# kokkos/kokkos-kernels

Hardware: NVIDIA B200
Metric: spmv_fp64_gflops (higher is better)
Workload: dtype f64

## Files before the change

include/b200sparse.h:

```cpp
#ifndef B200SPARSE_H_
#define B200SPARSE_H_

#include <stdint.h>

#ifdef __cplusplus
extern "C" {
#endif

typedef enum {
  B200SP_OK = 0,
  B200SP_ERR_INVALID_ARGUMENT = 1,
  B200SP_ERR_CUDA = 2,
  B200SP_ERR_STATE = 3,
  B200SP_ERR_OVERFLOW = 4,
  B200SP_ERR_ALLOC = 5
} b200sp_status;

typedef enum {
  B200SP_SPMV_DEFAULT = 0,
  B200SP_SPMV_FAST_SETUP = 1,
  B200SP_SPMV_MERGE_PATH = 2
} b200sp_spmv_algo;

typedef struct b200sp_spmv_plan b200sp_spmv_plan;
// ... 248 lines not shown
int b200sp_gmres_bsr_f64_i32(b200sp_bsr_plan* plan_A, void* stream, int mb, int64_t nnzb, int bs, const int* row_ptr,
                             const int* col_idx, const double* vals, b200sp_bsr_plan* plan_M, int64_t nnzb_M,
                             const int* row_ptr_M, const int* col_idx_M, const double* vals_M, const double* b, double* x,
                             int m, double tol, int max_restart, int ortho, int* num_iters, double* end_rel_res,
                             int* conv_flag);
int b200sp_gmres_bsr_f32_i32(b200sp_bsr_plan* plan_A, void* stream, int mb, int64_t nnzb, int bs, const int* row_ptr,
                             const int* col_idx, const float* vals, b200sp_bsr_plan* plan_M, int64_t nnzb_M,
                             const int* row_ptr_M, const int* col_idx_M, const float* vals_M, const float* b, float* x, int m,
                             float tol, int max_restart, int ortho, int* num_iters, float* end_rel_res, int* conv_flag);

int64_t b200sp_launch_count(void);
const char* b200sp_spmv_last_kernel(const b200sp_spmv_plan* plan);
int b200sp_spmv_plan_invalidate(b200sp_spmv_plan* plan, void* stream);

int b200sp_spmv_plan_tune(b200sp_spmv_plan* plan, int cfg, int lanes_per_row, int ctas_per_sm);
#ifdef __cplusplus
}
#endif
#endif
```

kokkos-kernels_b200/_lib.py:

```python
import ctypes as C
import os

HERE = os.path.dirname(os.path.abspath(__file__))
LIBDIR = os.path.join(HERE, "lib")
SPARSE_SO = os.path.join(LIBDIR, "libb200sparse.so")
MATGEN_SO = os.path.join(LIBDIR, "libb200matgen.so")

i32, i64, f32, f64, vp, cp = C.c_int, C.c_int64, C.c_float, C.c_double, C.c_void_p, C.c_char
u64 = C.c_uint64

SPARSE_API = {
    "b200sp_last_error_string": (C.c_char_p, []),
    "b200sp_version": (i32, []),
    "b200sp_device_ok": (i32, []),
    "b200sp_spmv_plan_create": (i32, [C.POINTER(vp), i32]),
    "b200sp_spmv_plan_destroy": (i32, [vp, vp]),
    "b200sp_spmv_plan_set_option": (i32, [vp, i32, i32]),
    "b200sp_spmv_f64_i32": (i32, [vp, vp, cp, i32, i32, i64, f64, vp, vp, vp, vp, f64, vp]),
    "b200sp_spmv_f32_i32": (i32, [vp, vp, cp, i32, i32, i64, f32, vp, vp, vp, vp, f32, vp]),
    "b200sp_gs2_plan_create": (i32, [C.POINTER(vp)]),
    "b200sp_gs2_plan_destroy": (i32, [vp, vp]),
    "b200sp_gs2_plan_set": (i32, [vp, i32, f64]),
    "b200sp_gs2_symbolic_i32": (i32, [vp, vp, i32, i32, vp, vp]),
    "b200sp_gs2_numeric_f64_i32": (i32, [vp, vp, i32, i32, vp, vp, vp, vp]),
# ... 8 lines not shown
    "b200sp_sptrsv_solve_f64_i32": (i32, [vp, vp, i32, vp, vp, vp, vp, vp]),
    "b200sp_sptrsv_solve_f32_i32": (i32, [vp, vp, i32, vp, vp, vp, vp, vp]),
    "b200sp_spmv_hostvec_flush": (i32, [vp, vp]),
    "b200sp_spmv64_plan_create": (i32, [C.POINTER(vp), i32]),
    "b200sp_spmv64_plan_destroy": (i32, [vp, vp]),
    "b200sp_spmv64_plan_set_window": (i32, [vp, i64]),
    "b200sp_spmv64_plan_windows": (i32, [vp]),
    "b200sp_spmv64_last_kernel": (C.c_char_p, [vp]),
    "b200sp_spmv_f64_i64": (i32, [vp, vp, cp, i64, i64, i64, f64, vp, vp, i32, vp, vp, f64, vp]),
    "b200sp_spmv_f32_i64": (i32, [vp, vp, cp, i64, i64, i64, f32, vp, vp, i32, vp, vp, f32, vp]),
    "b200sp_spmm_f64_i64": (i32, [vp, vp, cp, i64, i64, i64, i32, f64, vp, vp, i32, vp, vp, i64, i32, f64, vp, i64, i32]),
    "b200sp_spmm_f32_i64": (i32, [vp, vp, cp, i64, i64, i64, i32, f32, vp, vp, i32, vp, vp, i64, i32, f32, vp, i64, i32]),
    "b200sp_spmv_scatter_f64_i32": (i32, [vp, vp, i32, i32, i64, f64, vp, vp, vp, vp, vp, i32, C.POINTER(vp)]),
    "b200sp_spmv_forward_f64_i32": (i32, [vp, vp, i32, i32, i64, f64, vp, vp, vp, vp, vp, vp]),
    "b200sp_spmv_plan_invalidate": (i32, [vp, vp]),
    "b200sp_peer_push": (i32, [vp, vp, i64, i32, C.POINTER(vp)]),
    "b200sp_peer_push_async": (i32, [vp, C.POINTER(vp), i32, C.POINTER(vp), vp, i64]),
    "b200sp_peer_join": (i32, [vp, C.POINTER(vp), i32]),
    "b200sp_multicast_push": (i32, [vp, vp, vp, i64, i32]),
    "b200sp_peer_push_sm": (i32, [vp, vp, i64, i32, C.POINTER(vp), i32]),
    "b200sp_spmv_hostvec_f64_i32": (i32, [vp, vp, cp, i32, i32, i64, f64, vp, vp, vp, vp, f64, vp]),
    "b200sp_spmm_f64_i32": (i32, [vp, vp, cp, i32, i32, i64, i32, f64, vp, vp, vp, vp, i64, i32, f64, vp, i64, i32]),
    "b200sp_spmm_f32_i32": (i32, [vp, vp, cp, i32, i32, i64, i32, f32, vp, vp, vp, vp, i64, i32, f32, vp, i64, i32]),
    "b200sp_spgemm_plan_create": (i32, [C.POINTER(vp)]),
    "b200sp_spgemm_plan_destroy": (i32, [vp, vp]),
    "b200sp_spgemm_symbolic_i32": (i32, [vp, vp, i32, i32, i32, vp, vp, vp, vp, vp, C.POINTER(i64), C.POINTER(i32)]),
    "b200sp_spgemm_numeric_f64_i32": (i32, [vp, vp, i32, i32, i32, vp, vp, vp, vp, vp, vp, vp, vp, vp]),
    "b200sp_spgemm_numeric_f32_i32": (i32, [vp, vp, i32, i32, i32, vp, vp, vp, vp, vp, vp, vp, vp, vp]),
    "b200sp_spgemm_jacobi_f64_i32": (i32, [vp, vp, i32, i32, i32, vp, vp, vp, vp, vp, vp, vp, vp, vp, f64, vp]),
    "b200sp_spgemm_jacobi_f32_i32": (i32, [vp, vp, i32, i32, i32, vp, vp, vp, vp, vp, vp, vp, vp, vp, f32, vp]),
# ... 112 lines not shown
```

kokkos-kernels_b200/csrc/spmv.cu:

```cuda
#include "common.cuh"
#include "tile_ring.cuh"
#include "spmm_items.h"
#include <stdarg.h>
#include <stdlib.h>
#include <string.h>
#include <algorithm>
#include <mutex>

namespace b200sp {

static thread_local char g_err[512] = "";
std::atomic<long long> g_launches{0};

void set_error(const char* fmt, ...) {
  va_list ap;
  va_start(ap, fmt);
  vsnprintf(g_err, sizeof(g_err), fmt, ap);
  va_end(ap);
}

int sm_count() {
  static int cached[64];
  static std::once_flag once;
  std::call_once(once, [] { memset(cached, 0, sizeof(cached)); });
// ... 449 lines not shown
          }
#pragma unroll
          for (int u = 0; u < UNR; ++u) xv[u] = (j0 + u * LPR < jend) ? ldg(x + c[u]) : S(0);
#pragma unroll
          for (int u = 0; u < UNR; ++u) sum += av[u] * xv[u];
        }
        sum = subwarp_sum<LPR>(sum);
        if (valid && !is_long && sl == 0) store_y(y, r, sum, alpha, beta, ex);
      }
      __syncwarp();
      if (lane == 0) mbar_arrive(&sm.empty[stage]);
    }
  }
}

struct TileCfg {
  int cap, stages, nw;
};
static const TileCfg kCfgs[] = {
    {2048, 4, 8},
    {4096, 4, 16},
    {4096, 3, 8},
    {1024, 6, 8},
    {2048, 3, 16},
    {2048, 3, 24},
    {2048, 3, 31},
    {1024, 5, 16},
    {2048, 4, 16},
    {2048, 3, 16},
    {4096, 3, 31},
// ... 92 lines not shown
  int algo = B200SP_SPMV_DEFAULT;
  int cfg = -1, lpr = -1, ctas_per_sm = -1;
  const int* key_row_ptr = nullptr;
  int key_m = -1, key_n = -1;
  int64_t key_nnz = -1;
  int key_cfg = -1;
  int4* tiles = nullptr;
  int n_tiles = 0;
  int T = 0, LMAX = 0;
  int* long_rows = nullptr;
  int* n_long = nullptr;
  int* n_long_host = nullptr;
  cudaEvent_t n_long_event = nullptr;
  bool n_long_known = false;
  int long_cap = 0;
  void* dx = nullptr;
  void* dy = nullptr;
  size_t dx_bytes = 0, dy_bytes = 0;
  void* xt = nullptr;
  void* yt = nullptr;
  size_t xt_bytes = 0, yt_bytes = 0;
  int* chunk_row = nullptr;
  int n_chunks = 0, chunk_q = 0;
  const int* chunk_key = nullptr;
  int chunk_m = -1;
  int64_t chunk_nnz = -1;
  int4* r1_segs = nullptr;
  int* r1_n_seg = nullptr;
  int2* r1_row_seg = nullptr;
  void* r1_partial = nullptr;
// ... 53 lines not shown
  if (p->r1_segs) cudaFreeAsync(p->r1_segs, st);
  if (p->r1_n_seg) cudaFreeAsync(p->r1_n_seg, st);
  if (p->r1_row_seg) cudaFreeAsync(p->r1_row_seg, st);
  if (p->r1_partial) cudaFreeAsync(p->r1_partial, st);
  p->r1_segs = nullptr;
  p->r1_n_seg = nullptr;
  p->r1_row_seg = nullptr;
  p->r1_partial = nullptr;
  p->r1_built = false;
  p->tiles = nullptr;
  p->long_rows = nullptr;
  p->n_long = nullptr;
  p->n_tiles = 0;
  p->n_long_known = false;
  p->key_row_ptr = nullptr;
}

static void plan_release_mm(b200sp_spmv_plan* p, cudaStream_t st) {
  void* ptrs[] = {p->mm_tiles, p->mm_long_rows, p->mm_n_long, p->mm_segs, p->mm_n_seg};
  for (void* q : ptrs)
    if (q) cudaFreeAsync(q, st);
  p->mm_tiles = nullptr;
  p->mm_long_rows = nullptr;
  p->mm_n_long = nullptr;
  p->mm_segs = nullptr;
  p->mm_n_seg = nullptr;
  p->mm_key_row_ptr = nullptr;
  void* iptrs[] = {p->mmi.items, p->mmi.multi, p->mmi.partial};
  for (void* q : iptrs)
    if (q) cudaFreeAsync(q, st);
  p->mmi = b200sp::MMItems();
}

b200sp::MMItems* plan_mm_items(b200sp_spmv_plan* p) { return &p->mmi; }

template <typename S>
static int plan_analyse(b200sp_spmv_plan* p, cudaStream_t st, int cfg, int m, int n, int64_t nnz,
                        const int* row_ptr) {
  if (p->key_row_ptr == row_ptr && p->key_m == m && p->key_n == n && p->key_nnz == nnz &&
      p->key_cfg == cfg && p->tiles)
    return B200SP_OK;
  plan_release_analysis(p, st);
  const TileCfg c = kCfgs[cfg];
  p->LMAX = c.cap / 4;
  p->T = c.cap - p->LMAX - 8;
  p->n_tiles = (int)(nnz / p->T) + 1;
  p->long_cap = (int)(nnz / (p->LMAX + 1)) + 1;
  B200SP_CUDA_TRY(cudaMallocAsync((void**)&p->tiles, sizeof(int4) * (size_t)p->n_tiles, st));
  B200SP_CUDA_TRY(cudaMallocAsync((void**)&p->long_rows, sizeof(int) * (size_t)p->long_cap, st));
  B200SP_CUDA_TRY(cudaMallocAsync((void**)&p->n_long, sizeof(int), st));
  B200SP_CUDA_TRY(cudaMemsetAsync(p->n_long, 0, sizeof(int), st));
  build_tiles_kernel<<<(p->n_tiles + 255) / 256, 256, 0, st>>>(m, row_ptr, p->n_tiles, p->T, c.cap, p->tiles);
  B200SP_LAUNCH_CHECK();
  find_long_rows_kernel<<<std::max(1, std::min((m + 255) / 256, sm_count() * 8)), 256, 0, st>>>(m, row_ptr, p->LMAX,
                                                                                                p->long_rows, p->n_long);
  B200SP_LAUNCH_CHECK();
  if (!p->n_long_host) B200SP_CUDA_TRY(cudaMallocHost((void**)&p->n_long_host, sizeof(int)));
  if (!p->n_long_event) B200SP_CUDA_TRY(cudaEventCreateWithFlags(&p->n_long_event, cudaEventDisableTiming));
  *p->n_long_host = -1;
  B200SP_CUDA_TRY(cudaMemcpyAsync(p->n_long_host, p->n_long, sizeof(int), cudaMemcpyDeviceToHost, st));
  B200SP_CUDA_TRY(cudaEventRecord(p->n_long_event, st));
  p->n_long_known = false;
  p->key_row_ptr = row_ptr;
  p->key_m = m;
  p->key_n = n;
  p->key_nnz = nnz;
  p->key_cfg = cfg;
  p->at_calls = 0;
  p->at_choice = -1;
  return B200SP_OK;
}

int plan_mv_scratch(b200sp_spmv_plan* p, cudaStream_t st, size_t xt_bytes, size_t yt_bytes, void** xt, void** yt) {
  if (xt_bytes > p->xt_bytes) {
    if (p->xt) cudaFreeAsync(p->xt, st);
    p->xt = nullptr;
    p->xt_bytes = 0;
    B200SP_CUDA_TRY(cudaMallocAsync(&p->xt, xt_bytes, st));
// ... 126 lines not shown
      kf<<<grid, (NW + 1) * 32, smem, st>>>(m, nnz, hi - lo, p->LMAX, p->tiles + lo, row_ptr, col_idx, vals, x, y, alpha, beta,
                                            p->extra);
      launched = true;
    }
  }
  if (!launched)
    kern<<<grid, (NW + 1) * 32, smem, st>>>(m, nnz, hi - lo, p->LMAX, p->tiles + lo, row_ptr, col_idx, vals, x, y,
                                            alpha, beta, direct_extra(p->extra));
  B200SP_LAUNCH_CHECK();
  snprintf(p->last_kernel, sizeof(p->last_kernel), "tile<%s,LPR=%d,NW=%d,STAGES=%d,CAP=%d,UNR=%d>grid=%d",
           sizeof(S) == 8 ? "f64" : "f32", LPR, NW, STAGES, CAP, UNR, grid);
  return B200SP_OK;
}

template <typename S, int LPR>
static int launch_tile_cfg(b200sp_spmv_plan* p, int cfg, cudaStream_t st, int m, int64_t nnz,
                           const int* row_ptr, const int* col_idx, const S* vals, const S* x, S* y,
                           S alpha, S beta) {
  switch (cfg) {
    case 0: return launch_tile<S, LPR, 8, 4, 2048>(p, st, m, nnz, row_ptr, col_idx, vals, x, y, alpha, beta);
    case 1: return launch_tile<S, LPR, 16, 4, 4096>(p, st, m, nnz, row_ptr, col_idx, vals, x, y, alpha, beta);
    case 2: return launch_tile<S, LPR, 8, 3, 4096>(p, st, m, nnz, row_ptr, col_idx, vals, x, y, alpha, beta);
    case 3: return launch_tile<S, LPR, 8, 6, 1024>(p, st, m, nnz, row_ptr, col_idx, vals, x, y, alpha, beta);
    case 4: return launch_tile<S, LPR, 16, 3, 2048>(p, st, m, nnz, row_ptr, col_idx, vals, x, y, alpha, beta);
    case 5: return launch_tile<S, LPR, 24, 3, 2048>(p, st, m, nnz, row_ptr, col_idx, vals, x, y, alpha, beta);
    case 6: return launch_tile<S, LPR, 31, 3, 2048>(p, st, m, nnz, row_ptr, col_idx, vals, x, y, alpha, beta);
    case 7: return launch_tile<S, LPR, 16, 5, 1024>(p, st, m, nnz, row_ptr, col_idx, vals, x, y, alpha, beta);
    case 8: return launch_tile<S, LPR, 16, 4, 2048>(p, st, m, nnz, row_ptr, col_idx, vals, x, y, alpha, beta);
    case 9: return launch_tile<S, LPR, 16, 3, 2048, 4>(p, st, m, nnz, row_ptr, col_idx, vals, x, y, alpha, beta);
    case 10: return launch_tile<S, LPR, 31, 3, 4096>(p, st, m, nnz, row_ptr, col_idx, vals, x, y, alpha, beta);
// ... 126 lines not shown
      case 8: spmv_transpose_kernel<S, 8><<<blocks, 256, 0, st>>>(m, row_ptr, col_idx, vals, x, y, alpha); break;
      case 16: spmv_transpose_kernel<S, 16><<<blocks, 256, 0, st>>>(m, row_ptr, col_idx, vals, x, y, alpha); break;
      default: spmv_transpose_kernel<S, 32><<<blocks, 256, 0, st>>>(m, row_ptr, col_idx, vals, x, y, alpha); break;
    }
    B200SP_LAUNCH_CHECK();
    if (p) snprintf(p->last_kernel, sizeof(p->last_kernel), "transpose<%s,LPR=%d>", sizeof(S) == 8 ? "f64" : "f32", lpr);
    return B200SP_OK;
  }

  const bool aligned = (((uintptr_t)vals | (uintptr_t)col_idx | (uintptr_t)row_ptr) & 15u) == 0;
  const bool use_tile = p && p->algo != B200SP_SPMV_FAST_SETUP && aligned &&
                        (nnz >= 32768 || p->cfg >= 0);
  if (!use_tile) return launch_vector<S>(p, st, (p && p->lpr > 0) ? p->lpr : lpr_auto, m, row_ptr, col_idx, vals, x, y, alpha, beta);

  const int cfg = p->cfg >= 0 ? p->cfg : 8;
  int rc = plan_analyse<S>(p, st, cfg, m, n, nnz, row_ptr);
  if (rc) return rc;
  const int lpr = p->lpr > 0 ? p->lpr : lpr_auto;
  const bool autotune = p->cfg < 0 && p->range_hi < 0 && p->extra.n == 0 && getenv("B200SP_NO_AUTOTUNE") == nullptr;
  int phase = -1;
  bool use_vec = false;
  if (autotune) {
    if (p->at_choice < 0 && p->at_calls >= 3 && cudaEventQuery(p->at_ev[1]) == cudaSuccess &&
        cudaEventQuery(p->at_ev[3]) == cudaSuccess) {
      if (cudaEventElapsedTime(&p->at_tile_ms, p->at_ev[0], p->at_ev[1]) == cudaSuccess &&
          cudaEventElapsedTime(&p->at_vec_ms, p->at_ev[2], p->at_ev[3]) == cudaSuccess)
        p->at_choice = (p->at_vec_ms < 0.9f * p->at_tile_ms) ? 1 : 0;
    }
    if (p->at_calls == 1 || p->at_calls == 2) {
      phase = p->at_calls;
      for (int i = 0; i < 4; ++i)
        if (!p->at_ev[i]) B200SP_CUDA_TRY(cudaEventCreate(&p->at_ev[i]));
    }
    p->at_calls++;
    use_vec = phase == 2 || (phase < 0 && p->at_choice == 1);
    if (phase > 0) B200SP_CUDA_TRY(cudaEventRecord(p->at_ev[phase == 1 ? 0 : 2], st));
  }
  if (use_vec) {
    rc = launch_vector<S>(p, st, lpr, m, row_ptr, col_idx, vals, x, y, alpha, beta, p->LMAX);
  } else {
    switch (lpr) {
      case 2: rc = launch_tile_cfg<S, 2>(p, cfg, st, m, nnz, row_ptr, col_idx, vals, x, y, alpha, beta); break;
      case 4: rc = launch_tile_cfg<S, 4>(p, cfg, st, m, nnz, row_ptr, col_idx, vals, x, y, alpha, beta); break;
      case 8: rc = launch_tile_cfg<S, 8>(p, cfg, st, m, nnz, row_ptr, col_idx, vals, x, y, alpha, beta); break;
      case 16: rc = launch_tile_cfg<S, 16>(p, cfg, st, m, nnz, row_ptr, col_idx, vals, x, y, alpha, beta); break;
      case 32: rc = launch_tile_cfg<S, 32>(p, cfg, st, m, nnz, row_ptr, col_idx, vals, x, y, alpha, beta); break;
      default: set_error("bad lanes-per-row %d", lpr); return B200SP_ERR_INVALID_ARGUMENT;
    }
  }
  if (rc) return rc;
  if (!p->n_long_known && cudaEventQuery(p->n_long_event) == cudaSuccess) p->n_long_known = true;
  if (!(p->n_long_known && *p->n_long_host == 0) && (p->range_hi < 0 || p->range_lo == 0)) {
    const char* lr = getenv("B200SP_SPMV_LONGROWS");
    if (lr && lr[0] == 's') {
// ... 78 lines not shown
      if (p->pipe.dx[b]) cudaFree(p->pipe.dx[b]);
      if (p->pipe.dy[b]) cudaFree(p->pipe.dy[b]);
      cudaEventDestroy(p->pipe.ev_x[b]);
      cudaEventDestroy(p->pipe.ev_c[b]);
      cudaEventDestroy(p->pipe.ev_done[b]);
    }
    for (int c = 0; c < 8; ++c) cudaEventDestroy(p->pipe.ev_chunk[c]);
    cudaStreamDestroy(p->pipe.sH);
    cudaStreamDestroy(p->pipe.sD);
  }
  if (p->n_long_event) {
    cudaEventSynchronize(p->n_long_event);
    cudaEventDestroy(p->n_long_event);
  }
  if (p->n_long_host) cudaFreeHost(p->n_long_host);
  delete p;
  return B200SP_OK;
}

int b200sp_spmv_plan_set_option(b200sp_spmv_plan* p, int option, int value) {
  B200SP_REQUIRE(p != nullptr, "spmv_plan_set_option: null plan");
  switch (option) {
    case B200SP_SPMV_OPT_CACHE_TRANSPOSE: p->cache_transpose = value != 0; return B200SP_OK;
    case B200SP_SPMV_OPT_HOSTVEC_DEFER:
      if (p->pipe.defer && value == 0 && p->pipe.last_b >= 0) {
        set_error("spmv_plan_set_option: downloads are outstanding, call b200sp_spmv_hostvec_flush first");
        return B200SP_ERR_STATE;
      }
      p->pipe.defer = value != 0;
      return B200SP_OK;
// ... 22 lines not shown
int b200sp_spmv_plan_tune(b200sp_spmv_plan* p, int cfg, int lanes_per_row, int ctas_per_sm) {
  B200SP_REQUIRE(p != nullptr, "spmv_plan_tune: null plan");
  B200SP_REQUIRE(cfg >= -1 && cfg < kNumCfgs, "spmv_plan_tune: cfg %d out of range", cfg);
  B200SP_REQUIRE(lanes_per_row == -1 || lanes_per_row == 2 || lanes_per_row == 4 || lanes_per_row == 8 ||
                     lanes_per_row == 16 || lanes_per_row == 32,
                 "spmv_plan_tune: lanes_per_row %d not in {2,4,8,16,32}", lanes_per_row);
  B200SP_REQUIRE(ctas_per_sm >= -1 && ctas_per_sm <= 8, "spmv_plan_tune: ctas_per_sm %d out of range", ctas_per_sm);
  p->cfg = cfg;
  p->lpr = lanes_per_row;
  p->ctas_per_sm = ctas_per_sm;
  return B200SP_OK;
}

const char* b200sp_spmv_last_kernel(const b200sp_spmv_plan* p) { return p ? p->last_kernel : "none"; }

int b200sp_spmv_f64_i32(b200sp_spmv_plan* plan, void* stream, char mode, int m, int n, int64_t nnz, double alpha,
                        const int* row_ptr, const int* col_idx, const double* vals, const double* x, double beta,
                        double* y) {
  return spmv_impl<double>(plan, (cudaStream_t)stream, mode, m, n, nnz, alpha, row_ptr, col_idx, vals, x, beta, y);
}

int b200sp_spmv_f32_i32(b200sp_spmv_plan* plan, void* stream, char mode, int m, int n, int64_t nnz, float alpha,
                        const int* row_ptr, const int* col_idx, const float* vals, const float* x, float beta,
                        float* y) {
  return spmv_impl<float>(plan, (cudaStream_t)stream, mode, m, n, nnz, alpha, row_ptr, col_idx, vals, x, beta, y);
}

int b200sp_spmv_scatter_f64_i32(b200sp_spmv_plan* p, void* stream, int m, int n, int64_t nnz, double alpha,
                                const int* row_ptr, const int* col_idx, const double* vals, const double* x,
                                double* y, int n_extra, void* const* y_extra) {
// ... 156 lines not shown
  }
  if (xb > q.xb || yb > q.yb) {
    B200SP_CUDA_TRY(cudaDeviceSynchronize());
    for (int b = 0; b < 2; ++b) {
      if (q.dx[b]) cudaFree(q.dx[b]);
      if (q.dy[b]) cudaFree(q.dy[b]);
      q.dx[b] = q.dy[b] = nullptr;
      B200SP_CUDA_TRY(cudaMalloc(&q.dx[b], std::max(xb, q.xb)));
      B200SP_CUDA_TRY(cudaMalloc(&q.dy[b], std::max(yb, q.yb)));
    }
    q.xb = std::max(xb, q.xb);
    q.yb = std::max(yb, q.yb);
    q.call = 0;
  }
  const int cfg = p->cfg >= 0 ? p->cfg : 8;
  int rc = plan_analyse<double>(p, st, cfg, m, n, nnz, row_ptr);
  if (rc) return rc;
  if (q.key != row_ptr || q.key_cfg != cfg || q.key_m != m || q.key_nnz != nnz || q.key_tiles != (const void*)p->tiles) {
    q.nc = 4;
    if (const char* e = getenv("B200SP_HOSTVEC_PIECES")) {
      const int v = atoi(e);
      if (v >= 1 && v <= 8) q.nc = v;
    }
    int4 d[9];
    for (int c = 0; c <= q.nc; ++c) {
      q.tile_b[c] = (int)(((int64_t)p->n_tiles * c) / q.nc);
      if (c < q.nc) B200SP_CUDA_TRY(cudaMemcpyAsync(&d[c], p->tiles + q.tile_b[c], sizeof(int4), cudaMemcpyDeviceToHost, st));
    }
    B200SP_CUDA_TRY(cudaStreamSynchronize(st));
    for (int c = 0; c < q.nc; ++c) q.row_b[c] = d[c].x;
    q.row_b[q.nc] = m;
// ... 56 lines not shown
```

kokkos-kernels_b200/sparse.py:

```python
import ctypes as C

import torch

from . import _lib
from ._lib import B200SparseError, B200SparseInvalidArgument, check

SPMV_DEFAULT, SPMV_FAST_SETUP, SPMV_NATIVE, SPMV_MERGE_PATH, SPMV_NATIVE_MERGE_PATH, SPMV_BSR_V41, SPMV_BSR_V42, SPMV_BSR_TC = range(8)
GS_DEFAULT, GS_PERMUTED, GS_TEAM, GS_CLUSTER, GS_TWOSTAGE = range(5)
SPGEMM_KK, SPGEMM_KK_MEMORY, SPGEMM_KK_SPEED, SPGEMM_KK_LP, SPGEMM_DEBUG, SPGEMM_SERIAL = range(6)

_ALGO_TO_C = {SPMV_DEFAULT: 0, SPMV_FAST_SETUP: 1, SPMV_NATIVE: 1, SPMV_MERGE_PATH: 2, SPMV_NATIVE_MERGE_PATH: 2, SPMV_BSR_V41: 0,
              SPMV_BSR_V42: 0, SPMV_BSR_TC: 0}


def _idx(t):
    if t is not None and t.dtype != torch.int32:
        raise B200SparseError(f"b200sparse: this operation takes int32 row maps / entries, got {t.dtype} "
                              "(only spmv accepts 64-bit offsets)")
    return _ptr(t)


def _ptr(t):
    return C.c_void_p(t.data_ptr()) if t is not None and t.numel() > 0 else C.c_void_p(0)

# ... 87 lines not shown
    def cache_transpose(self, enable=True):
        check(_lib.sparse().b200sp_spmv_plan_set_option(self._plan, 1, int(bool(enable))))

    def hostvec_defer(self, enable=True):
        check(_lib.sparse().b200sp_spmv_plan_set_option(self._plan, 2, int(bool(enable))))

    def hostvec_flush(self):
        check(_lib.sparse().b200sp_spmv_hostvec_flush(self._plan, _stream()))

    def tune(self, cfg=-1, lanes_per_row=-1, ctas_per_sm=-1):
        check(_lib.sparse().b200sp_spmv_plan_tune(self._plan, cfg, lanes_per_row, ctas_per_sm))

    def invalidate(self):
        if self._plan:
            check(_lib.sparse().b200sp_spmv_plan_invalidate(self._plan, _stream()))

    def last_kernel(self):
        if self._bsr_plan:
            return _lib.sparse().b200sp_bsr_last_kernel(self._bsr_plan).decode()
        if self._plan64:
            return _lib.sparse().b200sp_spmv64_last_kernel(self._plan64).decode()
        return _lib.sparse().b200sp_spmv_last_kernel(self._plan).decode()

    def __del__(self):
        try:
            st = _stream() if torch.cuda.is_available() else C.c_void_p(0)
            if self._bsr_plan:
                _lib.sparse().b200sp_bsr_plan_destroy(self._bsr_plan, st)
                self._bsr_plan = C.c_void_p(0)
            if self._plan64:
# ... 795 lines not shown
```

Measured before the change: 1023.

## Compress CSR column indices into per-row pattern dictionary for tiled SpMV

Adds an analysis pass that hashes each row's column offsets relative to the row index and builds a dictionary of the most frequent patterns held in shared memory. Each row then gets a 16-bit pattern ID. A new tile kernel streams these IDs in place of col_idx and rebuilds the columns from the dictionary, which cuts index bandwidth on structured (stencil-like) matrices. Rows that match no pattern fall back to reading col_idx. The costs are several setup kernels per plan, a larger shared-memory footprint, and a pattern path that only switches on once an async event reports that few nonzeros escaped.

```diff
diff --git a/include/b200sparse.h b/include/b200sparse.h
--- a/include/b200sparse.h
+++ b/include/b200sparse.h
@@ -286,6 +286,7 @@
 int b200sp_spmv_plan_invalidate(b200sp_spmv_plan* plan, void* stream);
 
 int b200sp_spmv_plan_tune(b200sp_spmv_plan* plan, int cfg, int lanes_per_row, int ctas_per_sm);
+int b200sp_spmv_plan_index_stats(b200sp_spmv_plan* plan, int64_t* out);
 #ifdef __cplusplus
 }
 #endif
diff --git a/kokkos-kernels_b200/_lib.py b/kokkos-kernels_b200/_lib.py
--- a/kokkos-kernels_b200/_lib.py
+++ b/kokkos-kernels_b200/_lib.py
@@ -46,6 +46,7 @@
     "b200sp_spmv_scatter_f64_i32": (i32, [vp, vp, i32, i32, i64, f64, vp, vp, vp, vp, vp, i32, C.POINTER(vp)]),
     "b200sp_spmv_forward_f64_i32": (i32, [vp, vp, i32, i32, i64, f64, vp, vp, vp, vp, vp, vp]),
     "b200sp_spmv_plan_invalidate": (i32, [vp, vp]),
+    "b200sp_spmv_plan_index_stats": (i32, [vp, C.POINTER(i64)]),
     "b200sp_peer_push": (i32, [vp, vp, i64, i32, C.POINTER(vp)]),
     "b200sp_peer_push_async": (i32, [vp, C.POINTER(vp), i32, C.POINTER(vp), vp, i64]),
     "b200sp_peer_join": (i32, [vp, C.POINTER(vp), i32]),
diff --git a/kokkos-kernels_b200/csrc/spmv.cu b/kokkos-kernels_b200/csrc/spmv.cu
--- a/kokkos-kernels_b200/csrc/spmv.cu
+++ b/kokkos-kernels_b200/csrc/spmv.cu
@@ -487,6 +487,382 @@
   }
 }
 
+constexpr int kPatSlots = 8192;
+constexpr int kPatProbes = 64;
+constexpr int kPatDictInts = 6144;
+constexpr int kPatMaxEscapeInv = 4;
+constexpr uint16_t kPatEscape = 0xFFFF;
+enum { kPatOff = 0, kPatPending = 1, kPatOn = 2 };
+
+struct PatInfo {
+  int use;
+  int overflow;
+  int npat;
+  int dict_ints;
+  unsigned long long esc_rows, esc_nnz;
+};
+
+__device__ __forceinline__ uint64_t row_pattern_key(const int* __restrict__ col_idx, int rs, int re, int r, uint64_t mask) {
+  uint64_t h = 0xcbf29ce484222325ull ^ (uint64_t)(uint32_t)(re - rs);
+  for (int j = rs; j < re; ++j) {
+    h ^= (uint64_t)((uint32_t)col_idx[j] - (uint32_t)r);
+    h *= 0x100000001b3ull;
+    h ^= h >> 29;
+  }
+  h ^= h >> 32;
+  h *= 0xbf58476d1ce4e5b9ull;
+  h ^= h >> 29;
+  return (h & mask) | (1ull << 63);
+}
+__device__ __forceinline__ int pat_slot(uint64_t key) { return (int)((key ^ (key >> 23)) & (kPatSlots - 1)); }
+
+__global__ void __launch_bounds__(256) pat_insert_kernel(int m, const int* __restrict__ row_ptr, const int* __restrict__ col_idx,
+                                                         int LMAX, uint64_t mask, unsigned long long* keys, unsigned* counts,
+                                                         int* reps, PatInfo* info) {
+  const int lane = threadIdx.x & 31;
+  const int64_t stride = (int64_t)gridDim.x * blockDim.x;
+  for (int64_t base = (int64_t)blockIdx.x * blockDim.x + (threadIdx.x & ~31); base < m; base += stride) {
+    int stop = 0;
+    if (lane == 0) stop = *(volatile int*)&info->overflow;
+    if (__shfl_sync(0xffffffffu, stop, 0)) return;
+    const int r = (int)base + lane;
+    int slot = -1;
+    if (r < m) {
+      const int rs = row_ptr[r], re = row_ptr[r + 1];
+      if (re - rs <= LMAX) {
+        const uint64_t key = row_pattern_key(col_idx, rs, re, r, mask);
+        int s = pat_slot(key);
+        for (int q = 0; q < kPatProbes; ++q, s = (s + 1) & (kPatSlots - 1)) {
+          unsigned long long k = *(volatile unsigned long long*)&keys[s];
+          if (k == 0ull) k = atomicCAS(&keys[s], 0ull, (unsigned long long)key);
+          if (k == 0ull || k == key) {
+            slot = s;
+            break;
+          }
+        }
+        if (slot < 0) *(volatile int*)&info->overflow = 1;
+      }
+    }
+    unsigned todo = __ballot_sync(0xffffffffu, slot >= 0);
+    while (todo) {
+      const int leader = __ffs((int)todo) - 1;
+      const int ls = __shfl_sync(0xffffffffu, slot, leader);
+      const unsigned same = __ballot_sync(0xffffffffu, slot == ls);
+      if (lane == leader) {
+        atomicAdd(&counts[ls], (unsigned)__popc(same));
+        atomicMin(&reps[ls], r);
+      }
+      todo &= ~same;
+    }
+  }
+}
+
+__global__ void __launch_bounds__(1024) pat_select_kernel(const int* __restrict__ row_ptr, const int* __restrict__ col_idx,
+                                                          const unsigned long long* __restrict__ keys,
+                                                          const unsigned* __restrict__ counts, const int* __restrict__ reps,
+                                                          int* __restrict__ slot_id, int* __restrict__ dict, PatInfo* info) {
+  extern __shared__ __align__(16) unsigned char pat_smem[];
+  unsigned long long* sk = reinterpret_cast<unsigned long long*>(pat_smem);
+  int* sv = reinterpret_cast<int*>(sk + kPatSlots);
+  int* spos = sv + kPatSlots;
+  __shared__ int n_occ, n_pat;
+  if (info->overflow) {
+    if (threadIdx.x == 0) info->npat = 0;
+    return;
+  }
+  if (threadIdx.x == 0) n_occ = 0;
+  __syncthreads();
+  for (int s = threadIdx.x; s < kPatSlots; s += blockDim.x)
+    if (keys[s] != 0ull) {
+      const int i = atomicAdd(&n_occ, 1);
+      sk[i] = ((unsigned long long)(0xffffffffu - counts[s]) << 32) | (unsigned)reps[s];
+      sv[i] = s;
+    }
+  __syncthreads();
+  const int n = n_occ;
+  int np2 = 1;
+  while (np2 < n) np2 <<= 1;
+  for (int i = n + threadIdx.x; i < np2; i += blockDim.x) {
+    sk[i] = ~0ull;
+    sv[i] = -1;
+  }
+  __syncthreads();
+  for (int k = 2; k <= np2; k <<= 1)
+    for (int j = k >> 1; j > 0; j >>= 1) {
+      for (int i = threadIdx.x; i < np2; i += blockDim.x) {
+        const int l = i ^ j;
+        if (l > i && ((sk[i] > sk[l]) == ((i & k) == 0))) {
+          const unsigned long long tk = sk[i];
+          sk[i] = sk[l];
+          sk[l] = tk;
+          const int tv = sv[i];
+          sv[i] = sv[l];
+          sv[l] = tv;
+        }
+      }
+      __syncthreads();
+    }
+  for (int i = threadIdx.x; i < n; i += blockDim.x) {
+    const int rep = (int)(unsigned)sk[i];
+    spos[i] = row_ptr[rep + 1] - row_ptr[rep];
+  }
+  __syncthreads();
+  if (threadIdx.x == 0) {
+    int np = 0, tot = 0;
+    while (np < n && np < (int)kPatEscape && (np + 2) + tot + spos[np] <= kPatDictInts) tot += spos[np++];
+    int pos = np + 1;
+    for (int i = 0; i < np; ++i) {
+      const int len = spos[i];
+      spos[i] = pos;
+      pos += len;
+    }
+    spos[np] = pos;
+    n_pat = np;
+    info->npat = np;
+    info->dict_ints = pos;
+  }
+  __syncthreads();
+  const int np = n_pat;
+  for (int i = threadIdx.x; i < np; i += blockDim.x) slot_id[sv[i]] = i;
+  for (int i = threadIdx.x; i <= np; i += blockDim.x) dict[i] = spos[i];
+  const int warp = threadIdx.x >> 5, lane = threadIdx.x & 31;
+  for (int i = warp; i < np; i += blockDim.x >> 5) {
+    const int rep = (int)(unsigned)sk[i];
+    const int rs = row_ptr[rep], p0 = spos[i], len = spos[i + 1] - p0;
+    for (int k = lane; k < len; k += 32) dict[p0 + k] = (int)((unsigned)col_idx[rs + k] - (unsigned)rep);
+  }
+}
+
+__global__ void __launch_bounds__(256) pat_assign_kernel(int m, const int* __restrict__ row_ptr, const int* __restrict__ col_idx,
+                                                         int LMAX, uint64_t mask, const unsigned long long* __restrict__ keys,
+                                                         const int* __restrict__ slot_id, const int* __restrict__ dict,
+                                                         uint16_t* __restrict__ ids, PatInfo* info) {
+  const int npat = info->npat;
+  if (npat == 0) return;
+  unsigned long long erows = 0, ennz = 0;
+  for (int r = blockIdx.x * blockDim.x + threadIdx.x; r < m; r += gridDim.x * blockDim.x) {
+    const int rs = row_ptr[r], re = row_ptr[r + 1], len = re - rs;
+    int id = -1;
+    if (len <= LMAX) {
+      const uint64_t key = row_pattern_key(col_idx, rs, re, r, mask);
+      int s = pat_slot(key);
+      for (int q = 0; q < kPatProbes; ++q, s = (s + 1) & (kPatSlots - 1)) {
+        const unsigned long long k = keys[s];
+        if (k == key) {
+          id = slot_id[s];
+          break;
+        }
+        if (k == 0ull) break;
+      }
+      if (id >= 0) {
+        const int p0 = dict[id];
+        if (dict[id + 1] - p0 != len) id = -1;
+        for (int k = 0; id >= 0 && k < len; ++k)
+          if (dict[p0 + k] != (int)((unsigned)col_idx[rs + k] - (unsigned)r)) id = -1;
+      }
+    }
+    ids[r] = id < 0 ? kPatEscape : (uint16_t)id;
+    if (id < 0) {
+      erows += 1;
+      ennz += (unsigned long long)len;
+    }
+  }
+  for (int o = 16; o > 0; o >>= 1) {
+    erows += __shfl_xor_sync(0xffffffffu, erows, o);
+    ennz += __shfl_xor_sync(0xffffffffu, ennz, o);
+  }
+  if ((threadIdx.x & 31) == 0 && erows) {
+    atomicAdd(&info->esc_rows, erows);
+    atomicAdd(&info->esc_nnz, ennz);
+  }
+}
+
+__global__ void pat_finish_kernel(int m, int64_t nnz, int force, PatInfo* info) {
+  if (info->npat == 0) {
+    info->use = 0;
+    info->esc_rows = (unsigned long long)m;
+    info->esc_nnz = (unsigned long long)nnz;
+    return;
+  }
+  info->use = (force || info->esc_nnz * kPatMaxEscapeInv <= (unsigned long long)nnz) ? 1 : 0;
+}
+
+template <typename S, int CAP, int STAGES>
+struct PatTileSmem {
+  static constexpr int RCAP = CAP / 2;
+  static constexpr int DICT = STAGES * CAP - STAGES * RCAP / 2;
+  alignas(128) S vals[STAGES][CAP];
+  alignas(128) int rows[STAGES][RCAP];
+  alignas(128) uint16_t ids[STAGES][RCAP];
+  alignas(16) int dict[DICT];
+  int4 desc[STAGES];
+  alignas(8) uint64_t full[STAGES];
+  alignas(8) uint64_t empty[STAGES];
+};
+
+template <int LPR, int UNR, typename S, typename Col>
+__device__ __forceinline__ S tile_row_dot(int j0, int jend, const S* __restrict__ sv, const S* __restrict__ x, Col col) {
+  S sum = S(0);
+  for (; j0 < jend; j0 += UNR * LPR) {
+    int c[UNR];
+    S av[UNR], xv[UNR];
+#pragma unroll
+    for (int u = 0; u < UNR; ++u) {
+      const int j = j0 + u * LPR;
+      const bool ok = j < jend;
+      c[u] = ok ? col(j) : 0;
+      av[u] = ok ? sv[j] : S(0);
+    }
+#pragma unroll
+    for (int u = 0; u < UNR; ++u) xv[u] = (j0 + u * LPR < jend) ? ldg(x + c[u]) : S(0);
+#pragma unroll
+    for (int u = 0; u < UNR; ++u) sum += av[u] * xv[u];
+  }
+  return sum;
+}
+
+template <typename S, int LPR, int NW, int STAGES, int CAP, int UNR>
+__global__ void __launch_bounds__((NW + 1) * 32, 2)
+    spmv_tile_pat_kernel(int m, int64_t nnz, int n_tiles, int LMAX, const int4* __restrict__ tiles,
+                         const int* __restrict__ row_ptr, const int* __restrict__ col_idx, const uint16_t* __restrict__ ids,
+                         const int* __restrict__ dict, const PatInfo* __restrict__ info, const S* __restrict__ vals,
+                         const S* __restrict__ x, S* __restrict__ y, S alpha, S beta, YExtra ex) {
+  using Smem = PatTileSmem<S, CAP, STAGES>;
+  static_assert(Smem::DICT >= kPatDictInts, "dictionary does not fit the ring");
+  constexpr int RCAP = Smem::RCAP;
+  extern __shared__ __align__(128) unsigned char smem_raw[];
+  Smem& sm = *reinterpret_cast<Smem*>(smem_raw);
+
+  const int warp = threadIdx.x >> 5;
+  const int lane = threadIdx.x & 31;
+  const bool use = info->use != 0;
+
+  if (threadIdx.x == 0) {
+#pragma unroll
+    for (int s = 0; s < STAGES; ++s) {
+      mbar_init(&sm.full[s], 1);
+      mbar_init(&sm.empty[s], NW);
+    }
+    fence_mbar_init();
+  }
+  if (use) {
+    const int nd = info->dict_ints;
+    for (int i = threadIdx.x; i < nd; i += blockDim.x) sm.dict[i] = dict[i];
+  }
+  __syncthreads();
+
+  if (warp == NW) {
+    const uint64_t pol = l2_policy_evict_first();
+    const int64_t nnz_al = nnz & ~(int64_t)3;
+    const int rp_al_end = (m + 1) & ~3;
+    int4 mine = make_int4(0, 0, 0, 0);
+    for (int it = 0;; ++it) {
+      const int64_t tile = blockIdx.x + (int64_t)it * gridDim.x;
+      if (tile >= n_tiles) break;
+      if ((it & 31) == 0) {
+        const int64_t t = blockIdx.x + (int64_t)(it + lane) * gridDim.x;
+        if (t < n_tiles) mine = tiles[t];
+      }
+      int4 d;
+      d.x = __shfl_sync(0xffffffffu, mine.x, it & 31);
+      d.y = __shfl_sync(0xffffffffu, mine.y, it & 31);
+      d.z = __shfl_sync(0xffffffffu, mine.z, it & 31);
+      d.w = __shfl_sync(0xffffffffu, mine.w, it & 31);
+      const int stage = it % STAGES;
+      const uint32_t ph = (uint32_t)(it / STAGES) & 1u;
+      mbar_wait(&sm.empty[stage], ph ^ 1u);
+
+      const int r0 = d.x, r1 = d.y, s = d.z, e = d.w;
+      S* sv = sm.vals[stage];
+      int* sr = sm.rows[stage];
+      const int s_al = s & ~3;
+      const int e_up = (e + 3) & ~3;
+      const int bulk_end = (int)dmin64(e_up, nnz_al);
+      const int nb = (r1 > r0 && bulk_end > s_al) ? bulk_end - s_al : 0;
+      if (r1 > r0 && (int64_t)e > nnz_al) {
+        const int t0 = (int)dmax64(s_al, nnz_al);
+        for (int i = t0 + lane; i < e; i += 32) sv[i - s_al] = vals[i];
+      }
+      const int r0_al = r0 & ~3;
+      int nrp = 0;
+      if (r1 > r0) {
+        const int want_end = min(r1 + 1, r0_al + RCAP);
+        const int want_up = (want_end + 3) & ~3;
+        const int rbulk_end = min(min(want_up, r0_al + RCAP), rp_al_end);
+        nrp = rbulk_end > r0_al ? rbulk_end - r0_al : 0;
+        if (want_end > rp_al_end) {
+          const int t0 = max(r0_al, rp_al_end);
+          for (int i = t0 + lane; i < want_end; i += 32) sr[i - r0_al] = row_ptr[i];
+        }
+      }
+      const int r0_a8 = r0 & ~7;
+      const int nid = (use && r1 > r0) ? min((r1 - r0_a8 + 7) & ~7, RCAP) : 0;
+      __syncwarp();
+      if (lane == 0) {
+        sm.desc[stage] = d;
+        mbar_arrive_expect_tx(&sm.full[stage], (uint32_t)(nb * sizeof(S) + nrp * 4 + nid * 2));
+        if (nb > 0) bulk_g2s(sv, vals + s_al, (uint32_t)(nb * sizeof(S)), &sm.full[stage], pol);
+        if (nrp > 0) bulk_g2s(sr, row_ptr + r0_al, (uint32_t)(nrp * 4), &sm.full[stage], pol);
+        if (nid > 0) bulk_g2s(sm.ids[stage], ids + r0_a8, (uint32_t)(nid * 2), &sm.full[stage], pol);
+      }
+      __syncwarp();
+    }
+  } else {
+    constexpr int RPW = 32 / LPR;
+    const int sub = lane / LPR, sl = lane % LPR;
+    for (int it = 0;; ++it) {
+      const int64_t tile = blockIdx.x + (int64_t)it * gridDim.x;
+      if (tile >= n_tiles) break;
+      const int stage = it % STAGES;
+      const uint32_t ph = (uint32_t)(it / STAGES) & 1u;
+      mbar_wait(&sm.full[stage], ph);
+      const int4 d = sm.desc[stage];
+      const int r0 = d.x, r1 = d.y;
+      const int s_al = d.z & ~3;
+      const int r0_al = r0 & ~3;
+      const int r0_a8 = r0 & ~7;
+      const S* sv = sm.vals[stage];
+      const int* sr = sm.rows[stage];
+      const uint16_t* si = sm.ids[stage];
+      const int* cg = col_idx + s_al;
+      const int g_first = r0 / RPW;
+      int g = g_first + ((warp - g_first % NW) + NW) % NW;
+      for (; g * RPW < r1; g += NW) {
+        const int r = g * RPW + sub;
+        const bool valid = (r >= r0) && (r < r1);
+        int rs = 0, re = 0;
+        int id = kPatEscape;
+        if (valid) {
+          const int o = r - r0_al;
+          if (o + 1 < RCAP) {
+            rs = sr[o];
+            re = sr[o + 1];
+          } else {
+            rs = row_ptr[r];
+            re = row_ptr[r + 1];
+          }
+          if (use) id = (r - r0_a8 < RCAP) ? si[r - r0_a8] : ids[r];
+        }
+        const bool is_long = (re - rs) > LMAX;
+        if (is_long) re = rs;
+        const int jend = re - s_al;
+        const int j0 = rs + sl - s_al;
+        S sum;
+        if (id != kPatEscape) {
+          const int* pd = sm.dict + (sm.dict[id] - (rs - s_al));
+          sum = tile_row_dot<LPR, UNR>(j0, jend, sv, x, [&](int j) { return (int)((unsigned)r + (unsigned)pd[j]); });
+        } else {
+          sum = tile_row_dot<LPR, UNR>(j0, jend, sv, x, [&](int j) { return ldg(cg + j); });
+        }
+        sum = subwarp_sum<LPR>(sum);
+        if (valid && !is_long && sl == 0) store_y(y, r, sum, alpha, beta, ex);
+      }
+      __syncwarp();
+      if (lane == 0) mbar_arrive(&sm.empty[stage]);
+    }
+  }
+}
+
 struct TileCfg {
   int cap, stages, nw;
 };
@@ -609,6 +985,13 @@
   cudaEvent_t n_long_event = nullptr;
   bool n_long_known = false;
   int long_cap = 0;
+  int pat_state = 0;
+  const int* key_col_idx = nullptr;
+  uint16_t* pat_ids = nullptr;
+  int* pat_dict = nullptr;
+  b200sp::PatInfo* pat_info = nullptr;
+  b200sp::PatInfo* pat_info_host = nullptr;
+  cudaEvent_t pat_event = nullptr;
   void* dx = nullptr;
   void* dy = nullptr;
   size_t dx_bytes = 0, dy_bytes = 0;
@@ -692,6 +1075,14 @@
   p->n_tiles = 0;
   p->n_long_known = false;
   p->key_row_ptr = nullptr;
+  p->key_col_idx = nullptr;
+  void* pptrs[] = {p->pat_ids, p->pat_dict, p->pat_info};
+  for (void* q : pptrs)
+    if (q) cudaFreeAsync(q, st);
+  p->pat_ids = nullptr;
+  p->pat_dict = nullptr;
+  p->pat_info = nullptr;
+  p->pat_state = kPatOff;
 }
 
 static void plan_release_mm(b200sp_spmv_plan* p, cudaStream_t st) {
@@ -712,10 +1103,63 @@
 
 b200sp::MMItems* plan_mm_items(b200sp_spmv_plan* p) { return &p->mmi; }
 
+static int plan_analyse_patterns(b200sp_spmv_plan* p, cudaStream_t st, int m, int64_t nnz, const int* row_ptr,
+                                 const int* col_idx) {
+  const char* mode = getenv("B200SP_SPMV_INDEX");
+  if (mode && strcmp(mode, "csr") == 0) return B200SP_OK;
+  const int force = (mode && strcmp(mode, "pattern") == 0) ? 1 : 0;
+  uint64_t mask = ~0ull;
+  if (const char* hb = getenv("B200SP_SPMV_PATTERN_HASH_BITS")) {
+    const int b = atoi(hb);
+    if (b >= 0 && b < 64) mask = (1ull << b) - 1ull;
+  }
+  B200SP_CUDA_TRY(cudaMallocAsync((void**)&p->pat_ids, sizeof(uint16_t) * ((size_t)m + 8), st));
+  B200SP_CUDA_TRY(cudaMallocAsync((void**)&p->pat_dict, sizeof(int) * (size_t)kPatDictInts, st));
+  B200SP_CUDA_TRY(cudaMallocAsync((void**)&p->pat_info, sizeof(PatInfo), st));
+  B200SP_CUDA_TRY(cudaMemsetAsync(p->pat_ids, 0xFF, sizeof(uint16_t) * ((size_t)m + 8), st));
+  B200SP_CUDA_TRY(cudaMemsetAsync(p->pat_info, 0, sizeof(PatInfo), st));
+  DevTmp tmp(st);
+  unsigned long long* keys;
+  unsigned* counts;
+  int *reps, *slot_id;
+  B200SP_CUDA_TRY(tmp.alloc(&keys, kPatSlots));
+  B200SP_CUDA_TRY(tmp.alloc(&counts, kPatSlots));
+  B200SP_CUDA_TRY(tmp.alloc(&reps, kPatSlots));
+  B200SP_CUDA_TRY(tmp.alloc(&slot_id, kPatSlots));
+  B200SP_CUDA_TRY(cudaMemsetAsync(keys, 0, sizeof(unsigned long long) * kPatSlots, st));
+  B200SP_CUDA_TRY(cudaMemsetAsync(counts, 0, sizeof(unsigned) * kPatSlots, st));
+  B200SP_CUDA_TRY(cudaMemsetAsync(reps, 0x7F, sizeof(int) * kPatSlots, st));
+  B200SP_CUDA_TRY(cudaMemsetAsync(slot_id, 0xFF, sizeof(int) * kPatSlots, st));
+  const int blocks = std::max(1, std::min((m + 255) / 256, sm_count() * 8));
+  pat_insert_kernel<<<blocks, 256, 0, st>>>(m, row_ptr, col_idx, p->LMAX, mask, keys, counts, reps, p->pat_info);
+  B200SP_LAUNCH_CHECK();
+  const size_t sel_smem = (size_t)kPatSlots * (sizeof(unsigned long long) + sizeof(int)) + sizeof(int) * ((size_t)kPatSlots + 1);
+  B200SP_CUDA_TRY(cudaFuncSetAttribute(pat_select_kernel, cudaFuncAttributeMaxDynamicSharedMemorySize, (int)sel_smem));
+  pat_select_kernel<<<1, 1024, sel_smem, st>>>(row_ptr, col_idx, keys, counts, reps, slot_id, p->pat_dict, p->pat_info);
+  B200SP_LAUNCH_CHECK();
+  pat_assign_kernel<<<blocks, 256, 0, st>>>(m, row_ptr, col_idx, p->LMAX, mask, keys, slot_id, p->pat_dict, p->pat_ids,
+                                            p->pat_info);
+  B200SP_LAUNCH_CHECK();
+  pat_finish_kernel<<<1, 1, 0, st>>>(m, nnz, force, p->pat_info);
+  B200SP_LAUNCH_CHECK();
+  if (!p->pat_info_host) B200SP_CUDA_TRY(cudaMallocHost((void**)&p->pat_info_host, sizeof(PatInfo)));
+  if (!p->pat_event) B200SP_CUDA_TRY(cudaEventCreateWithFlags(&p->pat_event, cudaEventDisableTiming));
+  B200SP_CUDA_TRY(cudaMemcpyAsync(p->pat_info_host, p->pat_info, sizeof(PatInfo), cudaMemcpyDeviceToHost, st));
+  B200SP_CUDA_TRY(cudaEventRecord(p->pat_event, st));
+  p->pat_state = kPatPending;
+  return B200SP_OK;
+}
+
+static bool plan_pattern_active(b200sp_spmv_plan* p) {
+  if (p->pat_state == kPatPending && cudaEventQuery(p->pat_event) == cudaSuccess)
+    p->pat_state = p->pat_info_host->use ? kPatOn : kPatOff;
+  return p->pat_state != kPatOff;
+}
+
 template <typename S>
 static int plan_analyse(b200sp_spmv_plan* p, cudaStream_t st, int cfg, int m, int n, int64_t nnz,
-                        const int* row_ptr) {
-  if (p->key_row_ptr == row_ptr && p->key_m == m && p->key_n == n && p->key_nnz == nnz &&
+                        const int* row_ptr, const int* col_idx) {
+  if (p->key_row_ptr == row_ptr && p->key_col_idx == col_idx && p->key_m == m && p->key_n == n && p->key_nnz == nnz &&
       p->key_cfg == cfg && p->tiles)
     return B200SP_OK;
   plan_release_analysis(p, st);
@@ -739,7 +1183,11 @@
   B200SP_CUDA_TRY(cudaMemcpyAsync(p->n_long_host, p->n_long, sizeof(int), cudaMemcpyDeviceToHost, st));
   B200SP_CUDA_TRY(cudaEventRecord(p->n_long_event, st));
   p->n_long_known = false;
+  if (cfg == 8 && p->cfg < 0) {
+    if (int rc = plan_analyse_patterns(p, st, m, nnz, row_ptr, col_idx)) return rc;
+  }
   p->key_row_ptr = row_ptr;
+  p->key_col_idx = col_idx;
   p->key_m = m;
   p->key_n = n;
   p->key_nnz = nnz;
@@ -896,6 +1344,27 @@
 }
 
 template <typename S, int LPR>
+static int launch_tile_pat(b200sp_spmv_plan* p, cudaStream_t st, int m, int64_t nnz, const int* row_ptr, const int* col_idx,
+                           const S* vals, const S* x, S* y, S alpha, S beta) {
+  constexpr int NW = 16, STAGES = 4, CAP = 2048, UNR = 8;
+  auto kern = spmv_tile_pat_kernel<S, LPR, NW, STAGES, CAP, UNR>;
+  const size_t smem = sizeof(PatTileSmem<S, CAP, STAGES>) + 128;
+  static KernelSetup ks;
+  int occ_dev = 1;
+  if (int rc = kernel_setup(ks, kern, (NW + 1) * 32, smem, &occ_dev)) return rc;
+  const int per_sm = p->ctas_per_sm > 0 ? p->ctas_per_sm : occ_dev;
+  const int lo = p->range_hi < 0 ? 0 : p->range_lo;
+  const int hi = p->range_hi < 0 ? p->n_tiles : p->range_hi;
+  const int grid = std::max(1, std::min(hi - lo, sm_count() * per_sm));
+  kern<<<grid, (NW + 1) * 32, smem, st>>>(m, nnz, hi - lo, p->LMAX, p->tiles + lo, row_ptr, col_idx, p->pat_ids, p->pat_dict,
+                                          p->pat_info, vals, x, y, alpha, beta, direct_extra(p->extra));
+  B200SP_LAUNCH_CHECK();
+  snprintf(p->last_kernel, sizeof(p->last_kernel), "tile_pat<%s,LPR=%d,NW=%d,STAGES=%d,CAP=%d,UNR=%d>grid=%d",
+           sizeof(S) == 8 ? "f64" : "f32", LPR, NW, STAGES, CAP, UNR, grid);
+  return B200SP_OK;
+}
+
+template <typename S, int LPR>
 static int launch_tile_cfg(b200sp_spmv_plan* p, int cfg, cudaStream_t st, int m, int64_t nnz,
                            const int* row_ptr, const int* col_idx, const S* vals, const S* x, S* y,
                            S alpha, S beta) {
@@ -1052,7 +1521,7 @@
   if (!use_tile) return launch_vector<S>(p, st, (p && p->lpr > 0) ? p->lpr : lpr_auto, m, row_ptr, col_idx, vals, x, y, alpha, beta);
 
   const int cfg = p->cfg >= 0 ? p->cfg : 8;
-  int rc = plan_analyse<S>(p, st, cfg, m, n, nnz, row_ptr);
+  int rc = plan_analyse<S>(p, st, cfg, m, n, nnz, row_ptr, col_idx);
   if (rc) return rc;
   const int lpr = p->lpr > 0 ? p->lpr : lpr_auto;
   const bool autotune = p->cfg < 0 && p->range_hi < 0 && p->extra.n == 0 && getenv("B200SP_NO_AUTOTUNE") == nullptr;
@@ -1076,6 +1545,15 @@
   }
   if (use_vec) {
     rc = launch_vector<S>(p, st, lpr, m, row_ptr, col_idx, vals, x, y, alpha, beta, p->LMAX);
+  } else if (p->cfg < 0 && p->extra.n >= 0 && plan_pattern_active(p)) {
+    switch (lpr) {
+      case 2: rc = launch_tile_pat<S, 2>(p, st, m, nnz, row_ptr, col_idx, vals, x, y, alpha, beta); break;
+      case 4: rc = launch_tile_pat<S, 4>(p, st, m, nnz, row_ptr, col_idx, vals, x, y, alpha, beta); break;
+      case 8: rc = launch_tile_pat<S, 8>(p, st, m, nnz, row_ptr, col_idx, vals, x, y, alpha, beta); break;
+      case 16: rc = launch_tile_pat<S, 16>(p, st, m, nnz, row_ptr, col_idx, vals, x, y, alpha, beta); break;
+      case 32: rc = launch_tile_pat<S, 32>(p, st, m, nnz, row_ptr, col_idx, vals, x, y, alpha, beta); break;
+      default: set_error("bad lanes-per-row %d", lpr); return B200SP_ERR_INVALID_ARGUMENT;
+    }
   } else {
     switch (lpr) {
       case 2: rc = launch_tile_cfg<S, 2>(p, cfg, st, m, nnz, row_ptr, col_idx, vals, x, y, alpha, beta); break;
@@ -1184,6 +1662,11 @@
     cudaEventDestroy(p->n_long_event);
   }
   if (p->n_long_host) cudaFreeHost(p->n_long_host);
+  if (p->pat_event) {
+    cudaEventSynchronize(p->pat_event);
+    cudaEventDestroy(p->pat_event);
+  }
+  if (p->pat_info_host) cudaFreeHost(p->pat_info_host);
   delete p;
   return B200SP_OK;
 }
@@ -1236,6 +1719,21 @@
 
 const char* b200sp_spmv_last_kernel(const b200sp_spmv_plan* p) { return p ? p->last_kernel : "none"; }
 
+int b200sp_spmv_plan_index_stats(b200sp_spmv_plan* p, int64_t* out) {
+  B200SP_REQUIRE(p != nullptr && out != nullptr, "spmv_plan_index_stats: null argument");
+  for (int i = 0; i < 5; ++i) out[i] = 0;
+  if (p->pat_state == kPatOff && !p->pat_info) return B200SP_OK;
+  B200SP_CUDA_TRY(cudaEventSynchronize(p->pat_event));
+  plan_pattern_active(p);
+  const PatInfo& h = *p->pat_info_host;
+  out[0] = p->pat_state == kPatOn ? 1 : 0;
+  out[1] = h.npat;
+  out[2] = (int64_t)h.esc_rows;
+  out[3] = (int64_t)h.esc_nnz;
+  out[4] = p->pat_state == kPatOn ? (int64_t)sizeof(uint16_t) * p->key_m : 0;
+  return B200SP_OK;
+}
+
 int b200sp_spmv_f64_i32(b200sp_spmv_plan* plan, void* stream, char mode, int m, int n, int64_t nnz, double alpha,
                         const int* row_ptr, const int* col_idx, const double* vals, const double* x, double beta,
                         double* y) {
@@ -1422,7 +1920,7 @@
     q.call = 0;
   }
   const int cfg = p->cfg >= 0 ? p->cfg : 8;
-  int rc = plan_analyse<double>(p, st, cfg, m, n, nnz, row_ptr);
+  int rc = plan_analyse<double>(p, st, cfg, m, n, nnz, row_ptr, col_idx);
   if (rc) return rc;
   if (q.key != row_ptr || q.key_cfg != cfg || q.key_m != m || q.key_nnz != nnz || q.key_tiles != (const void*)p->tiles) {
     q.nc = 4;
diff --git a/kokkos-kernels_b200/sparse.py b/kokkos-kernels_b200/sparse.py
--- a/kokkos-kernels_b200/sparse.py
+++ b/kokkos-kernels_b200/sparse.py
@@ -125,6 +125,12 @@
     def invalidate(self):
         if self._plan:
             check(_lib.sparse().b200sp_spmv_plan_invalidate(self._plan, _stream()))
+
+    def index_stats(self):
+        out = (C.c_int64 * 5)()
+        check(_lib.sparse().b200sp_spmv_plan_index_stats(self._plan, out))
+        return {"format": "pattern" if out[0] else "csr", "patterns": int(out[1]), "escaped_rows": int(out[2]),
+                "escaped_nnz": int(out[3]), "id_bytes": int(out[4])}
 
     def last_kernel(self):
         if self._bsr_plan:
```

New measurement: 963.6, median of 6. 0.941x the previous value.
